# brunnergino/MIDI-VAE

Measured on AMD Instinct MI355X. Metric: MIDI roll windows/sec (train step), higher is better.
Workload: dtype bf16

## Files before the change

midi-vae_amd/csrc/heads.hip:

```cpp
#include "common.h"

namespace {

constexpr float CE_EPS = 1e-7f;

template <typename WT>
__device__ __forceinline__ typename op<WT>::frag frag_from(const float* src, bool valid);
template <>
__device__ __forceinline__ u16x8 frag_from<bf16_t>(const float* src, bool valid) {
    u16x8 v = {0, 0, 0, 0, 0, 0, 0, 0};
    if (valid) {
#pragma unroll
        for (int e = 0; e < 8; ++e) v[e] = f2bf(src[e]);
    }
    return v;
}
template <>
__device__ __forceinline__ f32x4 frag_from<float>(const float* src, bool valid) {
    return valid ? f32x4{src[0], src[1], src[2], src[3]} : f32x4{0.f, 0.f, 0.f, 0.f};
}

template <typename WT, int NTL, int KIND>
__host__ __device__ constexpr int head_rb() { return (sizeof(WT) == 2 && KIND == 0 && NTL <= 4) ? 2 : 1; }

template <typename WT, int NTL, int KIND>
__global__ __launch_bounds__(256) __attribute__((amdgpu_waves_per_eu(head_rb<WT, NTL, KIND>()))) void head_k(const mvae_head_args a) {
    constexpr int KG = op<WT>::KG, FE = op<WT>::FRAG_ELEMS;
    typedef typename op<WT>::frag frag;
    const int tid = threadIdx.x, w = tid >> 6, l = tid & 63, q = l >> 4, r = l & 15;
    const int R = a.R, H = a.H, N = a.N, NP = NTL * 16;
    const WT* __restrict__ hs = reinterpret_cast<const WT*>(a.hs);
    const WT* __restrict__ wt = reinterpret_cast<const WT*>(a.wt);
    float loss_acc = 0.0f, hit_acc = 0.0f;
    WT* __restrict__ dl = reinterpret_cast<WT*>(a.dlogits);
    constexpr int RB = head_rb<WT, NTL, KIND>();
    __shared__ __attribute__((aligned(16))) float stage[4 * RB * 16 * NTL * 16];
    __shared__ float wg_part[4][2];
    for (int row00 = (blockIdx.x * 4 + w) * 16 * RB; row00 < R; row00 += gridDim.x * 64 * RB) {
    f32x4 acc_[RB][NTL];
#pragma unroll
    for (int b = 0; b < RB; ++b)
#pragma unroll
        for (int n = 0; n < NTL; ++n) acc_[b][n] = f32x4{0.f, 0.f, 0.f, 0.f};
    for (int s = 0; s < H / KG; ++s) {
        frag fa[RB];
#pragma unroll
        for (int b = 0; b < RB; ++b)
            fa[b] = *reinterpret_cast<const frag*>(hs + (size_t)min(row00 + b * 16 + r, R - 1) * H + s * KG + q * FE);
#pragma unroll
        for (int n = 0; n < NTL; ++n) {
            const frag fb = *reinterpret_cast<const frag*>(wt + (size_t)(n * 16 + r) * H + s * KG + q * FE);
#pragma unroll
            for (int b = 0; b < RB; ++b) acc_[b][n] = op<WT>::mma(fa[b], fb, acc_[b][n]);
        }
    }
    float bias[NTL];
#pragma unroll
    for (int n = 0; n < NTL; ++n) bias[n] = (n * 16 + r < N) ? a.bias[n * 16 + r] : 0.0f;

#pragma unroll
    for (int b = 0; b < RB; ++b) {
    const int row0 = row00 + b * 16, wb = w * RB + b;
    const f32x4 (&acc)[NTL] = acc_[b];
#pragma unroll
    for (int i = 0; i < 4; ++i) {
        const int row = row0 + q * 4 + i;
        const bool rv = row < R;
        const bool counted = rv && (a.b_stride <= 0 || (row % a.b_stride) < a.b_valid);
        const int rc = rv ? row : R - 1;
        const float rw = a.row_weight ? a.row_weight[rc] : 1.0f;
        if (KIND == 0) {
            float lg[NTL], mx = -INFINITY;
#pragma unroll
            for (int n = 0; n < NTL; ++n) {
                lg[n] = (n * 16 + r < N) ? acc[n][i] + bias[n] : -INFINITY;
                mx = fmaxf(mx, lg[n]);
            }
            mx = group16_max(mx);
            float p[NTL], sum = 0.0f;
#pragma unroll
            for (int n = 0; n < NTL; ++n) {
                p[n] = __builtin_amdgcn_exp2f((lg[n] - mx) * 1.4426950408889634f);
                sum += p[n];
            }
            sum = group16_sum(sum);
            const float inv = 1.0f / sum;
            const int tg = a.target_idx ? (int)a.target_idx[rc] : 255;
            const int tg2 = a.target_idx2 ? (int)a.target_idx2[rc] : 255;
            float pt = 0.0f, pm = 0.0f, pt2 = 0.0f;
#pragma unroll
            for (int n = 0; n < NTL; ++n) {
                p[n] *= inv;
                pm = fmaxf(pm, p[n]);
                if (n * 16 + r == tg) pt = p[n];
                if (n * 16 + r == tg2) pt2 = p[n];
            }
            pt = group16_sum(pt);
            if (a.target_idx2) pt2 = group16_sum(pt2);
            pm = group16_max(pm);
            int am = 1 << 30;
#pragma unroll
            for (int n = 0; n < NTL; ++n)
                if (p[n] == pm && n * 16 + r < N) am = min(am, n * 16 + r);
            am = group16_min_i(am);
            const bool has_t = tg < N, has_t2 = tg2 < N;
            const bool inside = has_t && pt >= CE_EPS && pt <= 1.0f - CE_EPS;
            const bool inside2 = has_t2 && pt2 >= CE_EPS && pt2 <= 1.0f - CE_EPS;
            float ce = has_t ? -0.6931471805599453f * __builtin_amdgcn_logf(fminf(fmaxf(pt, CE_EPS), 1.0f - CE_EPS)) : 0.0f;
            if (has_t2) ce += -0.6931471805599453f * __builtin_amdgcn_logf(fminf(fmaxf(pt2, CE_EPS), 1.0f - CE_EPS));
            const int tfirst = has_t ? (has_t2 ? min(tg, tg2) : tg) : (has_t2 ? tg2 : 0);
            if (rv && r == 0) {
                loss_acc += rw * ce;
                hit_acc += (counted && am == tfirst) ? 1.0f : 0.0f;
                if (a.argmax) a.argmax[row] = (uint8_t)am;
            }
            if (rv) {
#pragma unroll
                for (int n = 0; n < NTL; ++n) {
                    const int col = n * 16 + r;
                    if (a.probs && col < N) a.probs[(size_t)row * N + col] = p[n];
                    if (a.want_grad) {
                        float g = inside ? a.grad_scale * rw * (p[n] - (col == tg ? 1.0f : 0.0f)) : 0.0f;
                        if (inside2) g += a.grad_scale * rw * (p[n] - (col == tg2 ? 1.0f : 0.0f));
                        stage[(wb * 16 + q * 4 + i) * NP + col] = col < N ? g : 0.0f;
                    }
                }
            }
        } else {
            const float pr = sigmoid_f(acc[0][i] + bias[0]);
            const float y = a.target_val ? a.target_val[rc] : 0.0f;
            if (rv && r == 0) {
                loss_acc += rw * (pr - y) * (pr - y);
                const float rounded = rintf(pr);
                hit_acc += (counted && rounded == y) ? 1.0f : 0.0f;
                if (a.probs) a.probs[row] = pr;
                if (a.argmax) a.argmax[row] = (uint8_t)rounded;
                if (a.want_grad) st<WT>::store(dl + (size_t)row * NP, a.grad_scale * rw * 2.0f * (pr - y) * pr * (1.0f - pr));
            }
            if (a.want_grad && a.dhs)
                stage[(wb * 16 + q * 4 + i) * NP + r] = (rv && r == 0) ? a.grad_scale * rw * 2.0f * (pr - y) * pr * (1.0f - pr) : 0.0f;
        }
    }
    if (KIND == 0 && a.want_grad) {
        __builtin_amdgcn_wave_barrier();
        asm volatile("s_waitcnt lgkmcnt(0)" ::: "memory");
        const float* mine = stage + wb * 16 * NP;
#pragma unroll
        for (int e = l * 4; e < 16 * NP; e += 256) {
            const int rr = e / NP, cc = e % NP;
            if (row0 + rr < R) st<WT>::store4(dl + (size_t)(row0 + rr) * NP + cc, *reinterpret_cast<const f32x4*>(mine + e));
        }
    }
    }
    if (a.want_grad && a.dhs) {
        if (KIND != 0) {
            __builtin_amdgcn_wave_barrier();
            asm volatile("s_waitcnt lgkmcnt(0)" ::: "memory");
        }
        const WT* __restrict__ wc = reinterpret_cast<const WT*>(a.wc);
        WT* __restrict__ dhs = reinterpret_cast<WT*>(a.dhs);
        f32x4 dacc[RB][16];
        const int HT = H >> 4;
#pragma unroll
        for (int b = 0; b < RB; ++b)
#pragma unroll
            for (int j = 0; j < 16; ++j) dacc[b][j] = f32x4{0.f, 0.f, 0.f, 0.f};
#pragma unroll
        for (int s2 = 0; s2 < (NP + KG - 1) / KG; ++s2) {
            const int k0 = s2 * KG + q * FE;
            const frag fz = frag_from<WT>(stage, false);
            frag fd[RB];
#pragma unroll
            for (int b = 0; b < RB; ++b)
                fd[b] = frag_from<WT>(stage + ((w * RB + b) * 16 + r) * NP + (k0 < NP ? k0 : 0), k0 < NP);
#pragma unroll
            for (int j = 0; j < 16; ++j) {
                if (j < HT) {
                    const frag fw = k0 < NP ? *reinterpret_cast<const frag*>(wc + (size_t)(j * 16 + r) * NP + k0) : fz;
#pragma unroll
                    for (int b = 0; b < RB; ++b)
                        dacc[b][j] = op<WT>::mma(fw, fd[b], dacc[b][j]);
                }
            }
        }
#pragma unroll
        for (int b = 0; b < RB; ++b) {
            const int row0 = row00 + b * 16;
            if (row0 < R) {
#pragma unroll
                for (int j = 0; j < 16; ++j)
                    if (j < HT)
                        st<WT>::store4(dhs + ((((size_t)(row0 >> 4) * HT + j) * 64) + (size_t)(q * 16 + r)) * 4, dacc[b][j]);
            }
        }
    }
        __builtin_amdgcn_wave_barrier();
    }
    if (a.scalars) {
        loss_acc = wave_sum(loss_acc);
        hit_acc = wave_sum(hit_acc);
        if (l == 0) {
            wg_part[w][0] = loss_acc;
            wg_part[w][1] = hit_acc;
        }
        __syncthreads();
        if (tid == 0) {
            atomicAdd(a.scalars, wg_part[0][0] + wg_part[1][0] + wg_part[2][0] + wg_part[3][0]);
            atomicAdd(a.scalars + 1, wg_part[0][1] + wg_part[1][1] + wg_part[2][1] + wg_part[3][1]);
        }
    }
}

template <typename WT, int KIND>
int launch(const mvae_head_args& a, hipStream_t s) {
    const int ntl = (a.N + 15) / 16;
    const dim3 block(256);
    auto grid = [&](int rb) {
        const int need = (a.R + 64 * rb - 1) / (64 * rb);
        const int cap = rb == 2 ? 512 : 1024;
        return dim3(need < cap ? need : cap);
    };
    switch (ntl) {
        case 1: hipLaunchKernelGGL((head_k<WT, 1, KIND>), grid(head_rb<WT, 1, KIND>()), block, 0, s, a); break;
        case 2: hipLaunchKernelGGL((head_k<WT, 2, KIND>), grid(head_rb<WT, 2, KIND>()), block, 0, s, a); break;
        case 3:
        case 4: hipLaunchKernelGGL((head_k<WT, 4, KIND>), grid(head_rb<WT, 4, KIND>()), block, 0, s, a); break;
        case 5: case 6: case 7:
        case 8: hipLaunchKernelGGL((head_k<WT, 8, KIND>), grid(head_rb<WT, 8, KIND>()), block, 0, s, a); break;
        default:
            if constexpr (KIND == 0) {
                if (ntl == 9) hipLaunchKernelGGL((head_k<WT, 9, KIND>), grid(1), block, 0, s, a);
                else if (ntl == 10) hipLaunchKernelGGL((head_k<WT, 10, KIND>), grid(1), block, 0, s, a);
                else if (ntl == 11) hipLaunchKernelGGL((head_k<WT, 11, KIND>), grid(1), block, 0, s, a);
                else if (ntl == 12) hipLaunchKernelGGL((head_k<WT, 12, KIND>), grid(1), block, 0, s, a);
                else return MVAE_E_UNSUPPORTED;
                break;
            }
            return MVAE_E_UNSUPPORTED;
    }
    MVAE_CHECK_LAUNCH();
    return MVAE_OK;
}

}

extern "C" int mvae_head_np(int32_t N) {
    const int ntl = (N + 15) / 16;
    if (ntl <= 1) return 16;
    if (ntl == 2) return 32;
    if (ntl <= 4) return 64;
    if (ntl <= 8) return 128;
    if (ntl <= 12) return ntl * 16;
    return -1;
}

extern "C" int mvae_head(const mvae_head_args* a, void* stream) {
    if (!a || !a->hs || !a->wt || !a->bias || a->R <= 0 || a->N <= 0 || a->H <= 0) return MVAE_E_ARG;
    if (a->kind != 0 && a->kind != 1) return MVAE_E_ARG;
    if (a->want_grad && !a->dlogits) return MVAE_E_ARG;
    if (a->dhs && (!a->wc || !a->want_grad || (a->R % 16) || (a->H % 16))) return MVAE_E_ARG;
    if (a->dhs && a->H > 256) return MVAE_E_UNSUPPORTED;
    if (a->kind == 1 && a->N != 1) return MVAE_E_ARG;
    if (a->kind == 0 && a->N > 192) return MVAE_E_UNSUPPORTED;
    hipStream_t s = reinterpret_cast<hipStream_t>(stream);
    if (a->dtype == MVAE_F32) {
        if (a->H % 16) return MVAE_E_UNSUPPORTED;
        return a->kind == 0 ? launch<float, 0>(*a, s) : launch<float, 1>(*a, s);
    }
    if (a->dtype == MVAE_BF16) {
        if (a->H % 32) return MVAE_E_UNSUPPORTED;
        return a->kind == 0 ? launch<bf16_t, 0>(*a, s) : launch<bf16_t, 1>(*a, s);
    }
    return MVAE_E_ARG;
}
```

Baseline: 39710.

## Stage head weights in LDS with 8-wave blocks and prefetch next hidden rows

Adds a weight-stationary variant of the output-head kernel. It copies the head weight fragments (and, for fused backward, the transpose weight fragments) into dynamic LDS once per block, runs 8 waves per block, and prefetches the next row tile's hidden-state fragments while finishing the current one. It also preloads row weights and targets ahead of the matmul. The aim is to stop re-reading the weights from global memory for every row tile and to hide hidden-state load latency. The cost is large LDS use that limits occupancy, plus extra registers for the prefetch buffers; when the LDS layout would exceed the cap, it falls back to the old path.

```diff
diff --git a/midi-vae_amd/csrc/heads.hip b/midi-vae_amd/csrc/heads.hip
--- a/midi-vae_amd/csrc/heads.hip
+++ b/midi-vae_amd/csrc/heads.hip
@@ -23,8 +23,25 @@
 template <typename WT, int NTL, int KIND>
 __host__ __device__ constexpr int head_rb() { return (sizeof(WT) == 2 && KIND == 0 && NTL <= 4) ? 2 : 1; }
 
+constexpr int HEAD_WS_WAVES = 8, HEAD_WS_PF = 8;
+constexpr size_t HEAD_WS_LDS_MAX = 160 * 1024 - 256;
+struct head_ws_lds {
+    int wt_frags, wc_frags;
+    size_t stage_off, bytes;
+};
 template <typename WT, int NTL, int KIND>
-__global__ __launch_bounds__(256) __attribute__((amdgpu_waves_per_eu(head_rb<WT, NTL, KIND>()))) void head_k(const mvae_head_args a) {
+__host__ __device__ inline head_ws_lds head_ws_layout(int H, bool grad, bool fused) {
+    constexpr int KG = op<WT>::KG, S2 = (NTL * 16 + KG - 1) / KG;
+    head_ws_lds o;
+    o.wt_frags = NTL * (H / KG) * 64;
+    o.wc_frags = fused ? (H >> 4) * S2 * 64 : 0;
+    o.stage_off = (size_t)(o.wt_frags + o.wc_frags) * 16;
+    o.bytes = o.stage_off + ((grad && (KIND == 0 || fused)) ? (size_t)HEAD_WS_WAVES * head_rb<WT, NTL, KIND>() * 16 * NTL * 16 * sizeof(float) : 0);
+    return o;
+}
+
+template <typename WT, int NTL, int KIND, bool WS>
+__global__ __launch_bounds__(WS ? 64 * HEAD_WS_WAVES : 256) __attribute__((amdgpu_waves_per_eu(head_rb<WT, NTL, KIND>()))) void head_k(const mvae_head_args a) {
     constexpr int KG = op<WT>::KG, FE = op<WT>::FRAG_ELEMS;
     typedef typename op<WT>::frag frag;
     const int tid = threadIdx.x, w = tid >> 6, l = tid & 63, q = l >> 4, r = l & 15;
@@ -34,14 +51,104 @@
     float loss_acc = 0.0f, hit_acc = 0.0f;
     WT* __restrict__ dl = reinterpret_cast<WT*>(a.dlogits);
     constexpr int RB = head_rb<WT, NTL, KIND>();
-    __shared__ __attribute__((aligned(16))) float stage[4 * RB * 16 * NTL * 16];
-    __shared__ float wg_part[4][2];
-    for (int row00 = (blockIdx.x * 4 + w) * 16 * RB; row00 < R; row00 += gridDim.x * 64 * RB) {
+    constexpr int WV = WS ? HEAD_WS_WAVES : 4;
+    constexpr int S2 = (NTL * 16 + KG - 1) / KG;
+    __shared__ __attribute__((aligned(16))) float stage_[WS ? 4 : 4 * RB * 16 * NTL * 16];
+    extern __shared__ __attribute__((aligned(16))) unsigned char ws_lds[];
+    __shared__ float wg_part[WV][2];
+    const bool fused = a.want_grad && a.dhs;
+    const int S = H / KG;
+    const head_ws_lds lay = head_ws_layout<WT, NTL, KIND>(H, a.want_grad, fused);
+    frag* const wl = reinterpret_cast<frag*>(ws_lds);
+    frag* const cl = wl + lay.wt_frags;
+    float* const stage = WS ? reinterpret_cast<float*>(ws_lds + lay.stage_off) : stage_;
+    float bias[NTL];
+    if constexpr (WS) {
+#pragma unroll
+        for (int n = 0; n < NTL; ++n) bias[n] = (n * 16 + r < N) ? a.bias[n * 16 + r] : 0.0f;
+        for (int g = tid; g < lay.wt_frags; g += 64 * WV) {
+            const int ll = g & 63, f = g >> 6, s = f % S, n = f / S;
+            wl[g] = *reinterpret_cast<const frag*>(wt + (size_t)(n * 16 + (ll & 15)) * H + s * KG + (ll >> 4) * FE);
+        }
+        if (fused) {
+            const WT* __restrict__ wc = reinterpret_cast<const WT*>(a.wc);
+            for (int g = tid; g < lay.wc_frags; g += 64 * WV) {
+                const int ll = g & 63, f = g >> 6, s2 = f % S2, j = f / S2, k0 = s2 * KG + (ll >> 4) * FE;
+                wl[lay.wt_frags + g] = k0 < NP ? *reinterpret_cast<const frag*>(wc + (size_t)(j * 16 + (ll & 15)) * NP + k0) : frag_from<WT>(nullptr, false);
+            }
+        }
+        __syncthreads();
+    }
+    const int stride = gridDim.x * WV * 16 * RB;
+    int row00 = (blockIdx.x * WV + w) * 16 * RB;
+    constexpr int PF = WS ? HEAD_WS_PF : 1;
+    const bool ahead = WS && S >= PF;
+    frag nx[RB][PF];
+    auto hs_frag = [&](int row0, int b, int s) {
+        return *reinterpret_cast<const frag*>(hs + (size_t)min(row0 + b * 16 + r, R - 1) * H + s * KG + q * FE);
+    };
+    auto request = [&](int row0) {
+#pragma unroll
+        for (int s = 0; s < PF; ++s)
+#pragma unroll
+            for (int b = 0; b < RB; ++b) nx[b][s] = hs_frag(row0, b, s);
+    };
+    if constexpr (WS) {
+        if (ahead && row00 < R) request(row00);
+    }
+    for (; row00 < R; row00 += stride) {
+    float rw_[RB][4], y_[RB][4];
+    int tg_[RB][4], tg2_[RB][4];
+    if constexpr (WS) {
+#pragma unroll
+        for (int b = 0; b < RB; ++b)
+#pragma unroll
+            for (int i = 0; i < 4; ++i) {
+                const int rc = min(row00 + b * 16 + q * 4 + i, R - 1);
+                const float rwv = *(a.row_weight ? a.row_weight + rc : a.bias);
+                rw_[b][i] = a.row_weight ? rwv : 1.0f;
+                if (KIND == 0) {
+                    const uint8_t* const none = reinterpret_cast<const uint8_t*>(a.hs);
+                    const int t1 = *(a.target_idx ? a.target_idx + rc : none), t2 = *(a.target_idx2 ? a.target_idx2 + rc : none);
+                    tg_[b][i] = a.target_idx ? t1 : 255;
+                    tg2_[b][i] = a.target_idx2 ? t2 : 255;
+                } else {
+                    const float yv = *(a.target_val ? a.target_val + rc : a.bias);
+                    y_[b][i] = a.target_val ? yv : 0.0f;
+                }
+            }
+    }
     f32x4 acc_[RB][NTL];
 #pragma unroll
     for (int b = 0; b < RB; ++b)
 #pragma unroll
         for (int n = 0; n < NTL; ++n) acc_[b][n] = f32x4{0.f, 0.f, 0.f, 0.f};
+    if constexpr (WS) {
+        auto group = [&](int s, const frag (&fa)[RB]) {
+#pragma unroll
+            for (int n = 0; n < NTL; ++n) {
+                const frag fb = wl[(n * S + s) * 64 + l];
+#pragma unroll
+                for (int b = 0; b < RB; ++b) acc_[b][n] = op<WT>::mma(fa[b], fb, acc_[b][n]);
+            }
+        };
+        if (ahead) {
+#pragma unroll
+            for (int s = 0; s < PF; ++s) {
+                frag fa[RB];
+#pragma unroll
+                for (int b = 0; b < RB; ++b) fa[b] = nx[b][s];
+                group(s, fa);
+            }
+        }
+        for (int s = ahead ? PF : 0; s < S; ++s) {
+            frag fa[RB];
+#pragma unroll
+            for (int b = 0; b < RB; ++b) fa[b] = hs_frag(row00, b, s);
+            group(s, fa);
+        }
+        if (ahead && row00 + stride < R) request(row00 + stride);
+    } else {
     for (int s = 0; s < H / KG; ++s) {
         frag fa[RB];
 #pragma unroll
@@ -54,9 +161,11 @@
             for (int b = 0; b < RB; ++b) acc_[b][n] = op<WT>::mma(fa[b], fb, acc_[b][n]);
         }
     }
-    float bias[NTL];
-#pragma unroll
-    for (int n = 0; n < NTL; ++n) bias[n] = (n * 16 + r < N) ? a.bias[n * 16 + r] : 0.0f;
+    }
+    if constexpr (!WS) {
+#pragma unroll
+        for (int n = 0; n < NTL; ++n) bias[n] = (n * 16 + r < N) ? a.bias[n * 16 + r] : 0.0f;
+    }
 
 #pragma unroll
     for (int b = 0; b < RB; ++b) {
@@ -68,7 +177,7 @@
         const bool rv = row < R;
         const bool counted = rv && (a.b_stride <= 0 || (row % a.b_stride) < a.b_valid);
         const int rc = rv ? row : R - 1;
-        const float rw = a.row_weight ? a.row_weight[rc] : 1.0f;
+        const float rw = WS ? rw_[b][i] : a.row_weight ? a.row_weight[rc] : 1.0f;
         if (KIND == 0) {
             float lg[NTL], mx = -INFINITY;
 #pragma unroll
@@ -85,8 +194,8 @@
             }
             sum = group16_sum(sum);
             const float inv = 1.0f / sum;
-            const int tg = a.target_idx ? (int)a.target_idx[rc] : 255;
-            const int tg2 = a.target_idx2 ? (int)a.target_idx2[rc] : 255;
+            const int tg = WS ? tg_[b][i] : a.target_idx ? (int)a.target_idx[rc] : 255;
+            const int tg2 = WS ? tg2_[b][i] : a.target_idx2 ? (int)a.target_idx2[rc] : 255;
             float pt = 0.0f, pm = 0.0f, pt2 = 0.0f;
 #pragma unroll
             for (int n = 0; n < NTL; ++n) {
@@ -128,7 +237,7 @@
             }
         } else {
             const float pr = sigmoid_f(acc[0][i] + bias[0]);
-            const float y = a.target_val ? a.target_val[rc] : 0.0f;
+            const float y = WS ? y_[b][i] : a.target_val ? a.target_val[rc] : 0.0f;
             if (rv && r == 0) {
                 loss_acc += rw * (pr - y) * (pr - y);
                 const float rounded = rintf(pr);
@@ -157,10 +266,36 @@
             __builtin_amdgcn_wave_barrier();
             asm volatile("s_waitcnt lgkmcnt(0)" ::: "memory");
         }
+        WT* __restrict__ dhs = reinterpret_cast<WT*>(a.dhs);
+        const int HT = H >> 4;
+        if constexpr (WS) {
+            frag fd[RB][S2];
+#pragma unroll
+            for (int s2 = 0; s2 < S2; ++s2) {
+                const int k0 = s2 * KG + q * FE;
+#pragma unroll
+                for (int b = 0; b < RB; ++b)
+                    fd[b][s2] = frag_from<WT>(stage + ((w * RB + b) * 16 + r) * NP + (k0 < NP ? k0 : 0), k0 < NP);
+            }
+#pragma unroll 4
+            for (int j = 0; j < HT; ++j) {
+                f32x4 d[RB];
+#pragma unroll
+                for (int b = 0; b < RB; ++b) d[b] = f32x4{0.f, 0.f, 0.f, 0.f};
+#pragma unroll
+                for (int s2 = 0; s2 < S2; ++s2) {
+                    const frag fw = cl[(j * S2 + s2) * 64 + l];
+#pragma unroll
+                    for (int b = 0; b < RB; ++b) d[b] = op<WT>::mma(fw, fd[b][s2], d[b]);
+                }
+#pragma unroll
+                for (int b = 0; b < RB; ++b)
+                    if (row00 + b * 16 < R)
+                        st<WT>::store4(dhs + ((((size_t)((row00 + b * 16) >> 4) * HT + j) * 64) + (size_t)(q * 16 + r)) * 4, d[b]);
+            }
+        } else {
         const WT* __restrict__ wc = reinterpret_cast<const WT*>(a.wc);
-        WT* __restrict__ dhs = reinterpret_cast<WT*>(a.dhs);
         f32x4 dacc[RB][16];
-        const int HT = H >> 4;
 #pragma unroll
         for (int b = 0; b < RB; ++b)
 #pragma unroll
@@ -192,6 +327,7 @@
                     if (j < HT)
                         st<WT>::store4(dhs + ((((size_t)(row0 >> 4) * HT + j) * 64) + (size_t)(q * 16 + r)) * 4, dacc[b][j]);
             }
+        }
         }
     }
         __builtin_amdgcn_wave_barrier();
@@ -205,41 +341,53 @@
         }
         __syncthreads();
         if (tid == 0) {
-            atomicAdd(a.scalars, wg_part[0][0] + wg_part[1][0] + wg_part[2][0] + wg_part[3][0]);
-            atomicAdd(a.scalars + 1, wg_part[0][1] + wg_part[1][1] + wg_part[2][1] + wg_part[3][1]);
-        }
-    }
+            float loss = wg_part[0][0], hits = wg_part[0][1];
+#pragma unroll
+            for (int v = 1; v < WV; ++v) {
+                loss += wg_part[v][0];
+                hits += wg_part[v][1];
+            }
+            atomicAdd(a.scalars, loss);
+            atomicAdd(a.scalars + 1, hits);
+        }
+    }
+}
+
+template <typename WT, int NTL, int KIND>
+int launch_tiles(const mvae_head_args& a, hipStream_t s) {
+    constexpr int rb = head_rb<WT, NTL, KIND>();
+    const head_ws_lds lay = head_ws_layout<WT, NTL, KIND>(a.H, a.want_grad != 0, a.want_grad && a.dhs);
+    if (lay.bytes <= HEAD_WS_LDS_MAX) {
+        const int need = (a.R + 16 * HEAD_WS_WAVES * rb - 1) / (16 * HEAD_WS_WAVES * rb);
+        const int cap = rb == 2 ? 256 : 512;
+        return mvae_launch<head_k<WT, NTL, KIND, true>>(dim3(need < cap ? need : cap), dim3(64 * HEAD_WS_WAVES), lay.bytes, s, a);
+    }
+    const int need = (a.R + 64 * rb - 1) / (64 * rb);
+    const int cap = rb == 2 ? 512 : 1024;
+    hipLaunchKernelGGL((head_k<WT, NTL, KIND, false>), dim3(need < cap ? need : cap), dim3(256), 0, s, a);
+    MVAE_CHECK_LAUNCH();
+    return MVAE_OK;
 }
 
 template <typename WT, int KIND>
 int launch(const mvae_head_args& a, hipStream_t s) {
     const int ntl = (a.N + 15) / 16;
-    const dim3 block(256);
-    auto grid = [&](int rb) {
-        const int need = (a.R + 64 * rb - 1) / (64 * rb);
-        const int cap = rb == 2 ? 512 : 1024;
-        return dim3(need < cap ? need : cap);
-    };
     switch (ntl) {
-        case 1: hipLaunchKernelGGL((head_k<WT, 1, KIND>), grid(head_rb<WT, 1, KIND>()), block, 0, s, a); break;
-        case 2: hipLaunchKernelGGL((head_k<WT, 2, KIND>), grid(head_rb<WT, 2, KIND>()), block, 0, s, a); break;
+        case 1: return launch_tiles<WT, 1, KIND>(a, s);
+        case 2: return launch_tiles<WT, 2, KIND>(a, s);
         case 3:
-        case 4: hipLaunchKernelGGL((head_k<WT, 4, KIND>), grid(head_rb<WT, 4, KIND>()), block, 0, s, a); break;
+        case 4: return launch_tiles<WT, 4, KIND>(a, s);
         case 5: case 6: case 7:
-        case 8: hipLaunchKernelGGL((head_k<WT, 8, KIND>), grid(head_rb<WT, 8, KIND>()), block, 0, s, a); break;
+        case 8: return launch_tiles<WT, 8, KIND>(a, s);
         default:
             if constexpr (KIND == 0) {
-                if (ntl == 9) hipLaunchKernelGGL((head_k<WT, 9, KIND>), grid(1), block, 0, s, a);
-                else if (ntl == 10) hipLaunchKernelGGL((head_k<WT, 10, KIND>), grid(1), block, 0, s, a);
-                else if (ntl == 11) hipLaunchKernelGGL((head_k<WT, 11, KIND>), grid(1), block, 0, s, a);
-                else if (ntl == 12) hipLaunchKernelGGL((head_k<WT, 12, KIND>), grid(1), block, 0, s, a);
-                else return MVAE_E_UNSUPPORTED;
-                break;
+                if (ntl == 9) return launch_tiles<WT, 9, KIND>(a, s);
+                if (ntl == 10) return launch_tiles<WT, 10, KIND>(a, s);
+                if (ntl == 11) return launch_tiles<WT, 11, KIND>(a, s);
+                if (ntl == 12) return launch_tiles<WT, 12, KIND>(a, s);
             }
             return MVAE_E_UNSUPPORTED;
     }
-    MVAE_CHECK_LAUNCH();
-    return MVAE_OK;
 }
 
 }
```

New measurement: 40070 (median of 5 runs). Within noise of the previous version (+0.9%).
